# nextpyp/cet_pick

Hardware: AMD Instinct MI355X
Metric: subtomograms/sec (MoCo-3D train) + voxels/sec (heatmap+NMS) at 1/2/4/8 GPU (higher is better)
Workload: dtype f32; 1 GPU; moco_main.py moco3d_18: 3D encoder, synthetic 512x512x128 tomogram, 32^3 subtomo crops, batch 64 per GPU, r=1024, dim=128, m=0.999, T=0.1, SGD lr 1e-3; global_batch=64, parallelism=dp1, hipgraph=True

## Files before the change

cet_pick_amd/_lib.py:

```python
import ctypes
import os

import torch

_HERE = os.path.dirname(os.path.abspath(__file__))
LIB_PATH = os.environ.get("CETPICK_HIP_LIB") or os.path.join(_HERE, "libcetpick_hip.so")

_c = ctypes
_P, _I, _F, _Z, _D, _L = _c.c_void_p, _c.c_int, _c.c_float, _c.c_size_t, _c.c_double, _c.c_long


class ConvGeom(ctypes.Structure):
    _fields_ = [(f, _I) for f in "N Di Hi Wi Ci Co kd kh kw stride pd ph pw dd dh dw".split()]


_G = _c.POINTER(ConvGeom)


class Aug2d3dRanges(ctypes.Structure):
    _fields_ = [(f, _F) for f in "flip_p angle_lo angle_hi erase_p scale_lo scale_hi ratio_lo ratio_hi".split()]


_R = _c.POINTER(Aug2d3dRanges)

# ... 32 lines not shown
    "mi_nms3d": (_I, [_P, _P, _I, _I, _I, _I, _I, _S]),
    "mi_decode_workspace_bytes": (_Z, [_I, _I, _I, _I]),
    "mi_decode_workspace_init": (_I, [_P, _Z, _S]),
    "mi_sigmoid_nms_topk": (_I, [_P, _P, _I, _I, _I, _I, _I, _I, _I, _P, _P, _P, _Z, _S]),
    "mi_gauss3d_sep": (_I, [_P, _P, _P, _I, _I, _I, _F, _S]),
    "mi_dog_pick_workspace_bytes": (_Z, [_I, _I, _I, _I]),
    "mi_dog_pick": (_I, [_P, _I, _I, _I, _P, _I, _I, _I, _I, _P, _P, _P, _P, _I, _P, _P, _Z, _S]),
    "mi_greedy_nms3d_workspace_bytes": (_Z, [_I, _I, _I]),
    "mi_greedy_nms3d": (_I, [_P, _I, _I, _I, _F, _F, _F, _P, _P, _P, _I, _P, _Z, _S]),
    "mi_crop_normalize": (_I, [_P, _I, _I, _I, _P, _I, _I, _I, _I, _I, _I, _P, _S]),
    "mi_crop_normalize_table": (_I, [_P, _P, _P, _P, _P, _c.c_int64, _I, _I, _I, _I, _I, _I, _P, _S]),
    "mi_u8_roundtrip_normalize": (_I, [_P, _P, _Z, _F, _F, _S]),
    "mi_aug2d_params": (_I, [_P, _c.c_int64, _c.c_uint64, _I, _I, _I] + [_F] * 7 + [_P, _S]),
    "mi_aug2d_apply": (_I, [_P, _c.c_int64, _I, _P, _P, _c.c_int64, _I, _F, _F, _P, _S]),
    "mi_aug2d3d_params": (_I, [_P, _c.c_int64, _c.c_uint64, _I, _I, _R, _R, _P, _S]),
    "mi_aug2d3d_apply": (_I, [_P, _P, _c.c_int64, _I, _P, _P, _P, _P, _c.c_int64, _I, _F, _F, _F, _F, _P, _S]),
    "mi_aug3d_params": (_I, [_P, _c.c_int64, _c.c_uint64, _I, _I, _I, _I, _R3, _P, _S]),
    "mi_aug3d_workspace_bytes": (_Z, [_c.c_int64, _I, _I]),
    "mi_aug3d_apply": (_I, [_P, _P, _P, _c.c_int64, _P, _P, _c.c_int64, _I, _I, _P, _P, _Z, _S]),
    "mi_tilt_patches": (_I, [_P, _I, _P, _P, _c.c_int64, _I, _I, _D, _D, _P, _P, _S]),
    "mi_semi_labels": (_I, [_P, _I, _I, _I, _P, _c.c_int64, _P, _I, _I, _S]),
    "mi_semi_pairs": (_I, [_P, _P, _I, _P, _P, _c.c_int64, _I, _I, _P, _P, _P, _S]),
    "mi_gauss2d_slices": (_I, [_P, _P, _P, _I, _I, _I, _F, _S]),
    "mi_rec_reorder": (_I, [_P, _I, _I, _I, _I, _I, _I, _P, _S]),
    "mi_vol_stats_workspace_bytes": (_Z, [_L, _L]),
    "mi_vol_stats": (_I, [_P, _L, _L, _P, _P, _Z, _S]),
    "mi_zscore": (_I, [_P, _P, _L, _L, _P, _S]),
    "mi_zscore_quantize_minmax": (_I, [_P, _P, _L, _L, _P, _D, _D, _I, _S]),
    "mi_conv_workspace_bytes": (_Z, [_G]),
    "mi_conv_fwd_f32": (_I, [_P, _P, _P, _P, _I, _I, _G, _P, _Z, _S]),
    "mi_conv_dgrad_f32": (_I, [_P, _P, _P, _P, _P, _G, _P, _Z, _S]),
    "mi_conv_wgrad_f32": (_I, [_P, _P, _P, _G, _P, _Z, _P, _S]),
    "mi_conv_wgrad_batch_f32": (_I, [_P, _P, _P, _P, _I, _G, _Z, _P, _S]),
    "mi_stem2d_fwd_bias_f32": (_I, [_P, _P, _P, _P, _I, _I, _I, _I, _S]),
    "mi_upconv_tail_fwd": (_I, [_P, _P, _P, _P, _P] + [_I] * 7 + [_S]),
    "mi_smallk_image_bytes": (_Z, [_I, _I]),
    "mi_smallk_prep": (_I, [_P, _P, _I, _I, _S]),
    "mi_smallk_fwd_f32": (_I, [_P, _P, _P, _P, _I, _L, _I, _I, _I, _L, _I, _S]),
    "mi_smallk_heads_fwd_f32": (_I, [_P, _P, _P, _P, _P, _I, _L, _I, _L, _I, _S]),
    "mi_splitk_reduce_batch": (_I, [_P, _P, _P, _P, _I, _S]),
    "mi_linear_fwd_f32": (_I, [_P, _P, _P, _P, _I, _I, _I, _P, _Z, _S]),
    "mi_conv3d_direct_wimg_bytes": (_Z, [_I]),
    "mi_conv3d_direct_workspace_bytes": (_Z, [_I, _I]),
    "mi_conv3d_direct_usable": (_I, [_I] * 9),
    "mi_conv3d_direct_prep": (_I, [_P, _P, _P, _P, _I, _S]),
    "mi_conv3d_direct_f32": (_I, [_P, _P, _P, _P, _P, _I, _I, _I, _I, _I, _I, _P, _Z, _S]),
    "mi_conv2d_p2d_usable": (_I, [_I] * 4),
    "mi_conv2d_p2d_wimg_bytes": (_Z, [_I]),
    "mi_conv2d_p2d_prep": (_I, [_P, _P, _P, _P, _I, _S]),
    "mi_conv2d_p2d_f32": (_I, [_P, _P, _P, _P, _P, _I, _I, _I, _I, _I, _S]),
    "mi_conv2d_p2d_wgrad_workspace_bytes": (_Z, [_I] * 4),
    "mi_conv2d_p2d_wgrad_f32": (_I, [_P, _P, _P, _I, _I, _I, _I, _P, _Z, _S]),
    "mi_conv2d_stem3_workspace_bytes": (_Z, [_I]),
    "mi_conv2d_stem3_fwd_f32": (_I, [_P, _P, _P, _I, _I, _I, _I, _S]),
    "mi_conv2d_stem3_wgrad_f32": (_I, [_P, _P, _P, _I, _I, _I, _I, _P, _Z, _S]),
    "mi_conv3d_cube2_workspace_bytes": (_Z, [_I, _I]),
    "mi_conv3d_cube2_usable": (_I, [_I] * 9),
    "mi_conv3d_cube2_f32": (_I, [_P, _P, _P, _P, _P, _I, _I, _I, _I, _P, _Z, _S]),
    "mi_conv_d32_kind": (_I, [_I] * 12),
    "mi_conv_d32_image_bytes": (_Z, [_I, _I]),
    "mi_conv_d64_image_bytes": (_Z, [_I, _I]),
    "mi_conv_d32_prep": (_I, [_P, _P, _I, _I, _S]),
    "mi_conv_d64_prep_co": (_I, [_P, _P, _I, _I, _I, _S]),
    "mi_conv_d32_1x1_fwd_f32": (_I, [_P, _P, _P, _P, _I, _I, _I, _I, _I, _I, _I, _S]),
    "mi_conv_d32_fwd_pool_f32": (_I, [_P, _P, _P, _P, _P] + [_I] * 7 + [_S]),
    "mi_conv_d32_fwd_pool_strided_f32": (_I, [_P, _P, _P, _P, _I, _P] + [_I] * 7 + [_S]),
# ... 245 lines not shown
```

cet_pick_amd/csrc/conv_direct3.hip:

```cpp
#include "common.h"
#include "bf16x3.h"
#include <type_traits>
#include <algorithm>

namespace {

using namespace bf3;

constexpr int C = 64;
constexpr int PLANE = 64;
constexpr int TZ = 2;
constexpr int PZ = TZ + 2;
constexpr int NV = PZ * PLANE;
constexpr int LEAD = 16;
constexpr int ZREC = 34;
constexpr int NREC = LEAD + NV + ZREC;
constexpr int ARR = NREC * 16;
constexpr int KS = C / 16;
constexpr int PL_BYTES = 2 * ARR;
constexpr int KS_BYTES = 3 * PL_BYTES;
constexpr int LDS_BYTES = KS * KS_BYTES;
constexpr int ZBASE = (LEAD + NV) * 16;
constexpr int WBLK = 1024;
constexpr int WSTEP = 2 * 3 * WBLK;
// ... 440 lines not shown
    u32x4 o[3];
    cut8(v, o);
    unsigned char* dst = img + (long)(((cb * KSn + ks) * NTAP + tap) * 2 + cw) * (3 * WBLK) + lane * 16;
    store_planes(dst, WBLK, o);
}
__global__ __launch_bounds__(256) void direct3_prep_kernel(PrepBatch b) {
    const int fmt = b.wide[blockIdx.y], idx = blockIdx.x * 256 + threadIdx.x;
    if (fmt == 1) { if (blockIdx.x < PREP_BLOCKS_WIDE) direct3s_prep_body(b.w[blockIdx.y], b.img[blockIdx.y], b.dgrad[blockIdx.y], idx); }
    else if (fmt == 2) { if (blockIdx.x < PREP_BLOCKS_WIDE) direct3_prep_body<128>(b.w[blockIdx.y], b.img[blockIdx.y], b.dgrad[blockIdx.y], idx); }
    else if (fmt == 3) direct3s256_prep_body(b.w[blockIdx.y], b.img[blockIdx.y], b.dgrad[blockIdx.y], idx);
    else if (blockIdx.x < PREP_BLOCKS) direct3_prep_body<C>(b.w[blockIdx.y], b.img[blockIdx.y], b.dgrad[blockIdx.y], idx);
}

constexpr int WG_SPLITS = 28;
constexpr int WROW = 64;
constexpr int WHALF = (PLANE + 1) * WROW;
constexpr int WPL = 2 * WHALF;
constexpr int WOP = 3 * WPL;
constexpr int WBUF = 2 * WOP;
constexpr int WZERO = PLANE * WROW;

constexpr int WG_MAXPROB = 4;
struct Direct3WgradParams {
    const float* x[WG_MAXPROB];
    const float* dy[WG_MAXPROB];
    float* slabs[WG_MAXPROB];
    int N, D;
    unsigned bytes;
    int nprob, splits;
    int H, W;
};

constexpr int W_HB = 3 * 2 * 8 * 128;
template <bool V4, int CT, bool TILED = false>
__global__ __launch_bounds__(512, 2) void direct3_wgrad_kernel(Direct3WgradParams p) {
    __shared__ __attribute__((aligned(16))) unsigned char lds[2 * WBUF + (TILED ? 2 * W_HB : 16)];
    unsigned char* const halo = lds + 2 * WBUF;
    static_assert(!TILED || (!V4 && CT == 64), "tiled planes: the 64-channel geometry");
    constexpr int NBLK = CT / 64;
    const int tid = threadIdx.x, lane = tid & 63;
    const int wave = __builtin_amdgcn_readfirstlane(tid >> 6);
    const int h = lane >> 5, l32 = lane & 31, i16 = lane & 15, g16 = (lane >> 4) & 1;
    const int kh = wave >> 2, wm = (wave >> 1) & 1, wn = wave & 1;
    const int per_grp = p.nprob * p.splits;
    const int grp = blockIdx.x / per_grp, rem = blockIdx.x % per_grp;
    const int pb = rem / p.splits, split = rem % p.splits, stride = p.splits;
    const int pair = grp % 9, chb = grp / 9;
    const int ci0 = (chb / NBLK) * 64, co0 = (chb % NBLK) * 64;
    const int dz = pair / 3, dy = pair % 3;
    const int tiles_x = TILED ? p.W >> 3 : 1, tiles = TILED ? (p.H >> 3) * tiles_x : 1;
    const int n_planes = p.N * p.D * tiles;

    const __amdgpu_buffer_rsrc_t xrs = rsrc(p.x[pb], p.bytes), yrs = rsrc(p.dy[pb], p.bytes);
    const int st_vox = tid >> 3, st_cg = tid & 7;
    const unsigned st_src = TILED ? 4u * (unsigned)(((st_vox >> 3) * p.W + (st_vox & 7)) * C + st_cg * 8)
                                  : 4u * (unsigned)(st_vox * CT + st_cg * 8);
    const int h_side = tid >> 8, h_row = (tid >> 5) & 7, h_c2 = tid & 31;
    const unsigned x_ch = 4u * (unsigned)ci0, y_ch = 4u * (unsigned)co0;
    const int zsh = V4 ? 0 : dz - 1;
    const int st_lds = (st_cg >> 2) * WHALF + st_vox * WROW + (st_cg & 3) * 16;
    auto next_plane = [&](int from) {
        if (V4) return from < n_planes ? from : -1;
        for (int pi = from; pi < n_planes; pi += stride) {
            const int zi = (pi / tiles) % p.D + dz - 1;
            if ((unsigned)zi < (unsigned)p.D) return pi;
        }
        return -1;
    };
    u32x4 ldx[2], ldy[2];
    u32x2 ldh = {0u, 0u};
    unsigned u_y, u_x, u_h;
    auto unit_offsets = [&](int pi) {
        if (pi < 0) { u_y = u_x = u_h = 0x80000000u; return; }
        if (!TILED) {
            u_y = 4u * (unsigned)((long)pi * PLANE * CT) + y_ch + st_src;
            u_x = 4u * (unsigned)((long)(pi + zsh) * PLANE * CT) + x_ch + st_src;
            u_h = 0x80000000u;
            return;
        }
        const int pl = pi / tiles, t = pi % tiles, y0 = (t / tiles_x) * 8, x0 = (t % tiles_x) * 8;
        u_y = 4u * (unsigned)((((long)pl * p.H + y0) * p.W + x0) * C) + st_src;
        const int xr = y0 + (st_vox >> 3) + dy - 1;
        u_x = (unsigned)xr < (unsigned)p.H
                  ? 4u * (unsigned)((((long)(pl + dz - 1) * p.H + xr) * p.W + x0 + (st_vox & 7)) * C + st_cg * 8) : 0x80000000u;
        const int hr = y0 + h_row + dy - 1, hc = h_side ? x0 + 8 : x0 - 1;
        u_h = ((unsigned)hr < (unsigned)p.H && (unsigned)hc < (unsigned)p.W)
                  ? 4u * (unsigned)((((long)(pl + dz - 1) * p.H + hr) * p.W + hc) * C + 2 * h_c2) : 0x80000000u;
    };
    auto stage_load = [&](int pi) {
        unit_offsets(pi);
        ldx[0] = __builtin_amdgcn_raw_buffer_load_b128(xrs, (int)u_x, 0, 0);
        ldx[1] = __builtin_amdgcn_raw_buffer_load_b128(xrs, (int)(u_x + 16u), 0, 0);
        ldy[0] = __builtin_amdgcn_raw_buffer_load_b128(yrs, (int)u_y, 0, 0);
        ldy[1] = __builtin_amdgcn_raw_buffer_load_b128(yrs, (int)(u_y + 16u), 0, 0);
        if (TILED) ldh = __builtin_amdgcn_raw_buffer_load_b64(xrs, (int)u_h, 0, 0);
    };
    unsigned hcu[3];
    auto halo_cut = [&]() {
        const unsigned a1 = rest(ldh[0]), b1 = rest(ldh[1]), a2 = rest(a1), b2 = rest(b1);
        hcu[0] = pack2(ldh[1], ldh[0]);
        hcu[1] = pack2(b1, a1);
        hcu[2] = pack2(b2, a2);
    };
    auto halo_store = [&](int buf) {
#pragma unroll
        for (int pl = 0; pl < 3; ++pl)
            *reinterpret_cast<unsigned*>(halo + buf * W_HB + ((pl * 2 + h_side) * 8 + h_row) * 128 + h_c2 * 4) = hcu[pl];
    };
    auto stage_store_unit = [&](int buf, int op) {
        float v[8];
#pragma unroll
        for (int e = 0; e < 4; ++e) {
// ... 1 lines not shown
            v[4 + e] = __uint_as_float(op ? ldy[1][e] : ldx[1][e]);
        }
        u32x4 o[3];
        cut8(v, o);
        unsigned char* dst = lds + buf * WBUF + op * WOP + st_lds;
#pragma unroll
        for (int pl = 0; pl < 3; ++pl) *reinterpret_cast<u32x4*>(dst + pl * WPL) = o[pl];
        if (TILED && op == 0) { halo_cut(); halo_store(buf); }
    };

    const int q4 = i16 >> 2;
    const int coloff = (16 * g16 + 4 * (i16 & 3)) * 2;
    const int b_base = wn * WHALF + (2 * kh * 16 + 8 * h + q4) * WROW + coloff;
    int a_sel[2][2];
#pragma unroll
    for (int lk = 0; lk < 2; ++lk)
#pragma unroll
        for (int hi = 0; hi < 2; ++hi) {
            const int v = 16 * (2 * kh + lk) + 8 * h + 4 * hi + q4;
            if (V4) {
                const int zi = (v >> 4) + dz - 1, yi = ((v >> 2) & 3) + dy - 1;
                a_sel[lk][hi] = wm * WHALF + (((unsigned)zi < 4u && (unsigned)yi < 4u) ? ((zi * 4 + yi) * 4 + (v & 3)) * WROW : WZERO) + coloff;
            } else if (TILED) {
                a_sel[lk][hi] = wm * WHALF + v * WROW + coloff;
            } else {
                const int yi = (v >> 3) + dy - 1;
                a_sel[lk][hi] = wm * WHALF + ((unsigned)yi < 8u ? (yi * 8 + (v & 7)) * WROW : WZERO) + coloff;
            }
        }
    int h_off[2];
#pragma unroll
    for (int lk = 0; lk < 2; ++lk) h_off[lk] = (2 * (2 * kh + lk) + h) * 128 + (32 * wm + l32) * 2;
    unsigned hl[2][2][3];

    f32x16 acc[3];
#pragma unroll
    for (int t = 0; t < 3; ++t)
#pragma unroll
        for (int r = 0; r < 16; ++r) acc[t][r] = 0.f;

    for (int i = tid; i < 2 * 2 * 3 * 2 * (WROW / 16); i += 512) {
        const int img = i / (WROW / 16), c16 = i % (WROW / 16);
        *reinterpret_cast<u32x4*>(lds + img * WHALF + WZERO + c16 * 16) = u32x4{0u, 0u, 0u, 0u};
    }

    int cur = next_plane(split);
    int nxt = cur >= 0 ? next_plane(cur + stride) : -1;
    stage_load(cur);
    if (cur >= 0) { stage_store_unit(0, 0); stage_store_unit(0, 1); }
    stage_load(nxt);
    __syncthreads();

    bf16x8 af[2][3][3], bfg[2][3];
    auto read_piece = [&](int buf, int lk, int j, auto SETc) {
        constexpr int SET = decltype(SETc)::value;
        const unsigned char* xb = lds + buf * WBUF;
        if (j < 3) {
            const unsigned char* yb = xb + WOP + b_base + lk * 16 * WROW + j * WPL;
            const bf16x4 lo = __builtin_amdgcn_ds_read_tr16_b64_v4bf16((lds_bf16x4*)(yb));
            const bf16x4 hi = __builtin_amdgcn_ds_read_tr16_b64_v4bf16((lds_bf16x4*)(yb + 4 * WROW));
            bfg[SET][j] = __builtin_shufflevector(lo, hi, 0, 1, 2, 3, 4, 5, 6, 7);
        } else {
            const int pl = j - 3;
            const bf16x4 lo = __builtin_amdgcn_ds_read_tr16_b64_v4bf16((lds_bf16x4*)(xb + pl * WPL + a_sel[lk][0]));
            const bf16x4 hi = __builtin_amdgcn_ds_read_tr16_b64_v4bf16((lds_bf16x4*)(xb + pl * WPL + a_sel[lk][1]));
            af[SET][1][pl] = __builtin_shufflevector(lo, hi, 0, 1, 2, 3, 4, 5, 6, 7);
            if (TILED) {
#pragma unroll
                for (int sd = 0; sd < 2; ++sd)
                    hl[SET][sd][pl] = *reinterpret_cast<const unsigned short*>(halo + buf * W_HB + ((pl * 2 + sd) * 8) * 128 + h_off[lk]);
// ... 11 lines not shown
    };
    auto derive = [&](int set, int dxv, int pl) {
        const u32x4 c = __builtin_bit_cast(u32x4, af[set][1][pl]);
        u32x4 o;
        if (dxv == 0) {
            o[0] = c[0] << 16;
#pragma unroll
            for (int j = 1; j < 4; ++j) o[j] = __builtin_amdgcn_alignbit(c[j], c[j - 1], 16);
            if (V4) o[2] &= HI16;
            if (TILED) o[0] |= hl[set][0][pl];
        } else {
#pragma unroll
            for (int j = 0; j < 3; ++j) o[j] = __builtin_amdgcn_alignbit(c[j + 1], c[j], 16);
            o[3] = c[3] >> 16;
            if (V4) o[1] &= 0x0000ffffu;
            if (TILED) o[3] |= hl[set][1][pl] << 16;
        }
        af[set][dxv][pl] = __builtin_bit_cast(bf16x8, o);
    };
    unsigned cu[3][8];
    auto cut_a = [&](int op, int e) {
        cu[0][e] = op ? ldy[e >> 2][e & 3] : ldx[e >> 2][e & 3];
        cu[1][e] = rest(cu[0][e]);
    };
    auto cut_b = [&](int e) { cu[2][e] = rest(cu[1][e]); };
    auto store_piece = [&](int buf, int op, int pl) {
        u32x4 o;
#pragma unroll
        for (int d = 0; d < 4; ++d) o[d] = pack2(cu[pl][2 * d + 1], cu[pl][2 * d]);
        *reinterpret_cast<u32x4*>(lds + buf * WBUF + op * WOP + st_lds + pl * WPL) = o;
    };

    int buf = 0;
    if (cur >= 0) {
#pragma unroll
        for (int i = 0; i < 3; ++i) read_pair(0, 0, i);
    }
    constexpr int DXO[3] = {1, 0, 2};
    while (cur >= 0) {
        const int nn = nxt >= 0 ? next_plane(nxt + stride) : -1;
        unit_offsets(nn);
        __builtin_amdgcn_sched_barrier(0);
#pragma unroll
        for (int lk = 0; lk < 2; ++lk) {
            const int op = lk;
#pragma unroll
            for (int m = 0; m < 18; ++m) {
                const int dxm = DXO[m / 6];
                acc[dxm] = __builtin_amdgcn_mfma_f32_32x32x16_bf16(af[lk][dxm][PA[m % 6]], bfg[lk][PB[m % 6]], acc[dxm], 0, 0, 0);
                if (m < 3) derive(lk, 0, m);
                if (m >= 6 && m < 9) derive(lk, 2, m - 6);
                if (m >= 2 && m < 10) cut_a(op, m - 2);
                if (m >= 3 && m < 11) cut_b(m - 3);
                if (m >= 11 && m < 14) store_piece(buf ^ 1, op, m - 11);
                if (lk == 1 && m >= 14) {
                    const int i = m - 14, hf = i & 1;
                    if (i < 2) ldx[hf] = __builtin_amdgcn_raw_buffer_load_b128(xrs, (int)(u_x + 16u * hf), 0, 0);
                    else ldy[hf] = __builtin_amdgcn_raw_buffer_load_b128(yrs, (int)(u_y + 16u * hf), 0, 0);
                    if (TILED && i == 3) ldh = __builtin_amdgcn_raw_buffer_load_b64(xrs, (int)u_h, 0, 0);
                }
                if (TILED && lk == 0 && m == 14) halo_cut();
                if (TILED && lk == 0 && m == 15) halo_store(buf ^ 1);
                if (lk == 0) {
                    if (m < 3) read_pair(buf, 1, m);
                } else {
                    if (m == 13) __syncthreads();
// ... 307 lines not shown
    MI_RETURN_IF_LAUNCH_FAILED();
    return MI_OK;
}
int mi_direct3h_launch(const float* a, const void* wimg, float* out, const float* res, const float* mask, int relu, int N,
                       int D, int H, int W, hipStream_t s) {
    Direct3hParams p = {a, (const unsigned char*)wimg, out, res, mask, relu, N, D, H, W, (unsigned)(4l * N * D * H * W * C)};
    hipLaunchKernelGGL(direct3h_kernel, dim3((unsigned)((long)N * (D / TZ) * ((H + 7) / 8) * ((W + 7) / 8))), dim3(256), 0, s, p);
    MI_RETURN_IF_LAUNCH_FAILED();
    return MI_OK;
}
int mi_direct3_launch128(const float* a, const void* wimg, float* out, const float* res, const float* mask, int relu, int N,
                         int D, hipStream_t s) {
    Direct3Params p = {a, (const unsigned char*)wimg, out, res, mask, relu, N, D, (unsigned)(4l * N * D * PLANE * 128)};
    hipLaunchKernelGGL((direct3_kernel<true, 128>), dim3((unsigned)(N * (D / TZ)), 2), dim3(256), 0, s, p);
    MI_RETURN_IF_LAUNCH_FAILED();
    return MI_OK;
}

int mi_direct3s_launch(const float* a, const void* wimg, float* out, const float* res, const float* mask, int relu, int N,
                       hipStream_t s) {
    Direct3sParams p = {a, (const unsigned char*)wimg, out, res, mask, relu, N, (unsigned)(4l * N * VS * CS)};
    hipLaunchKernelGGL(direct3s_kernel<CS>, dim3((unsigned)(4 * N)), dim3(256), 0, s, p);
    MI_RETURN_IF_LAUNCH_FAILED();
    return MI_OK;
}
int mi_direct3s_launch256(const float* a, const void* wimg, float* out, const float* res, const float* mask, int relu, int N,
                          hipStream_t s) {
    Direct3sParams p = {a, (const unsigned char*)wimg, out, res, mask, relu, N, (unsigned)(4l * N * VS * 256)};
    hipLaunchKernelGGL(direct3s_kernel<256>, dim3((unsigned)(8 * N)), dim3(256), 0, s, p);
    MI_RETURN_IF_LAUNCH_FAILED();
    return MI_OK;
}

size_t mi_direct3_wgrad_slab_bytes() { return sizeof(float) * (size_t)WG_SPLITS * NTAP * C * C; }
int mi_direct3_wgrad_splits() { return WG_SPLITS; }

int mi_direct3_wgrad_launch(const float* x, const float* dy, float* slabs, int N, int D, hipStream_t s) {
    Direct3WgradParams p = {};
    p.x[0] = x; p.dy[0] = dy; p.slabs[0] = slabs; p.N = N; p.D = D; p.bytes = (unsigned)(4l * N * D * PLANE * C);
    p.nprob = 1; p.splits = WG_SPLITS;
    hipLaunchKernelGGL((direct3_wgrad_kernel<false, 64>), dim3(9 * WG_SPLITS), dim3(512), 0, s, p);
    MI_RETURN_IF_LAUNCH_FAILED();
    return MI_OK;
}
int mi_direct3_wgrad_batch_max() { return WG_MAXPROB; }
constexpr int WG_BATCH_SPLITS = 7;
int mi_direct3_wgrad_batch_splits(int nb) {
    if (nb < 1 || nb > WG_MAXPROB) return 0;
    if (const char* v = getenv("MI_D3W_BATCH_SPLITS")) { const int sv = atoi(v); if (sv >= 1 && sv <= WG_SPLITS) return sv; }
    return WG_BATCH_SPLITS;
}
int mi_direct3_wgrad_launch_batch(const float* const* xs, const float* const* dys, float* const* slabs, int nb, int N, int D,
                                  hipStream_t s) {
    if (nb < 1 || nb > WG_MAXPROB) return MI_E_ARG;
    Direct3WgradParams p = {};
    for (int i = 0; i < nb; ++i) { p.x[i] = xs[i]; p.dy[i] = dys[i]; p.slabs[i] = slabs[i]; }
    p.N = N; p.D = D; p.bytes = (unsigned)(4l * N * D * PLANE * C);
    p.nprob = nb; p.splits = mi_direct3_wgrad_batch_splits(nb);
    hipLaunchKernelGGL((direct3_wgrad_kernel<false, 64>), dim3(9 * nb * p.splits), dim3(512), 0, s, p);
    MI_RETURN_IF_LAUNCH_FAILED();
    return MI_OK;
}

constexpr int WS_SPLITS = 7, WS_BATCH_SPLITS = 2;
size_t mi_direct3s_wgrad_slab_bytes() { return sizeof(float) * (size_t)WS_SPLITS * NTAP * CS * CS; }
int mi_direct3s_wgrad_splits(int nb) {
    if (nb < 1 || nb > WG_MAXPROB) return 0;
    if (nb == 1) return WS_SPLITS;
    if (const char* v = getenv("MI_D3SW_BATCH_SPLITS")) { const int sv = atoi(v); if (sv >= 1 && sv <= WS_SPLITS) return sv; }
    return WS_BATCH_SPLITS;
}
int mi_direct3s_wgrad_launch_batch(const float* const* xs, const float* const* dys, float* const* slabs, int nb, int N, hipStream_t s) {
    if (nb < 1 || nb > WG_MAXPROB || N < 1) return MI_E_ARG;
    Direct3WgradParams p = {};
    for (int i = 0; i < nb; ++i) { p.x[i] = xs[i]; p.dy[i] = dys[i]; p.slabs[i] = slabs[i]; }
    p.N = N; p.D = 1; p.bytes = (unsigned)(4l * N * PLANE * CS);
    p.nprob = nb; p.splits = mi_direct3s_wgrad_splits(nb);
    hipLaunchKernelGGL((direct3_wgrad_kernel<true, 128>), dim3(36 * nb * p.splits), dim3(512), 0, s, p);
    MI_RETURN_IF_LAUNCH_FAILED();
    return MI_OK;
}

int mi_direct3t_wgrad_launch(const float* x, const float* dy, float* slabs, int N, int D, int H, int W, hipStream_t s) {
    if (H % 8 || W % 8 || H < 8 || W < 8) return MI_E_UNSUPPORTED;
    Direct3WgradParams p = {};
    p.x[0] = x; p.dy[0] = dy; p.slabs[0] = slabs; p.N = N; p.D = D; p.H = H; p.W = W;
    p.bytes = (unsigned)(4l * N * D * H * W * C);
    p.nprob = 1; p.splits = WG_SPLITS;
    hipLaunchKernelGGL((direct3_wgrad_kernel<false, 64, true>), dim3(9 * WG_SPLITS), dim3(512), 0, s, p);
    MI_RETURN_IF_LAUNCH_FAILED();
    return MI_OK;
}
// ... 45 lines not shown
```

cet_pick_amd/csrc/conv_igemm.hip:

```cpp
#include "common.h"
#include "bf16x3.h"
#include <algorithm>
#include <cstdlib>
#include <type_traits>

int mi_stem7_fwd(const float* x, const float* w, float* y, const float* res, int relu, int N, int D, int H, int W,
                 int Co, int bf16x3, void* ws, size_t ws_bytes, hipStream_t s, double* sums = nullptr);
size_t mi_stem7_fwd_workspace_bytes();
size_t mi_stem7_fwd_stats_workspace_bytes(int N, int D, int H, int W);
size_t mi_stem7_wgrad_workspace_bytes(int N, int D, int H, int W, int Co);
int mi_stem7_wgrad(const float* x, const float* dy, float* dw, int N, int D, int H, int W, int Co, int bf16x3, void* ws,
                   size_t ws_bytes, hipStream_t s);

int mi_direct3_kind(int N, int Di, int Hi, int Wi, int Ci, int Co, int kd, int kh, int kw, int stride, int pd, int ph,
                    int pw, int dd, int dh, int dw);
size_t mi_direct3_wimg_bytes(int channels);
size_t mi_direct3_slab_bytes(int N, int channels);
int mi_direct3_prep(const float* const* w, void* const* img, const int* dgrad, const int* channels, int n, hipStream_t s);
int mi_direct3_launch(const float* a, const void* wimg, float* out, const float* res, const float* mask, int relu, int N,
                      int D, hipStream_t s);
size_t mi_direct3_wimg_bytes_kind(int kind);
int mi_direct3_prep_kind(const float* const* w, void* const* img, const int* dgrad, const int* kinds, int n, hipStream_t s);
int mi_direct3s_launch256(const float* a, const void* wimg, float* out, const float* res, const float* mask, int relu, int N,
                          hipStream_t s);
int mi_direct3h_launch(const float* a, const void* wimg, float* out, const float* res, const float* mask, int relu, int N,
                       int D, int H, int W, hipStream_t s);
int mi_direct3_launch128(const float* a, const void* wimg, float* out, const float* res, const float* mask, int relu, int N,
                         int D, hipStream_t s);
int mi_direct3s_launch(const float* a, const void* wimg, float* out, const float* res, const float* mask, int relu, int N,
                       hipStream_t s);
int mi_direct3_finish_slabs(const float* slabs, int n_slabs, long out_elems, float* out, const float* res, const float* mask,
                            int relu, hipStream_t s);
size_t mi_direct3_wgrad_slab_bytes();
int mi_direct3_wgrad_splits();
int mi_direct3_wgrad_launch(const float* x, const float* dy, float* slabs, int N, int D, hipStream_t s);
int mi_direct3_wgrad_batch_max();
int mi_direct3_wgrad_batch_splits(int nb);
int mi_direct3_wgrad_launch_batch(const float* const* xs, const float* const* dys, float* const* slabs, int nb, int N, int D, hipStream_t s);
size_t mi_direct3s_wgrad_slab_bytes();
int mi_direct3s_wgrad_splits(int nb);
int mi_direct3s_wgrad_launch_batch(const float* const* xs, const float* const* dys, float* const* slabs, int nb, int N, hipStream_t s);
int mi_direct3t_wgrad_launch(const float* x, const float* dy, float* slabs, int N, int D, int H, int W, hipStream_t s);
int mi_direct3x_wgrad_splits(int kind);
size_t mi_direct3x_wgrad_slab_bytes(int kind);
int mi_direct3x_wgrad_launch(int kind, const float* x, const float* dy, float* slabs, int N, int D, hipStream_t s);
int mi_pair_wgrad_batch_max();
int mi_pair_wgrad_launch_batch(const float* const* xs, const float* const* dys, float* const* dws, float* const* slabs, int nb, int N, int Di,
                               int Ci, int Co, int k, int stride, hipStream_t s);
bool mi_cube2_usable(int N, int Di, int Hi, int Wi, int Ci, int Co, int kd, int kh, int kw, int stride, int pd, int ph, int pw,
                     int dd, int dh, int dw);
size_t mi_cube2_slab_bytes(int N, int C);
int mi_cube2_splits();
int mi_cube2_launch(int dgrad, const float* a, const float* w, float* slabs, int N, int C, hipStream_t s, const Cube2Final* fin = nullptr);
bool mi_pair_wgrad_usable(int N, int Di, int Hi, int Wi, int Ci, int Co, int kd, int kh, int kw, int stride, int pd, int ph, int pw,
                          int dd, int dh, int dw);
int mi_pair_wgrad_splits(int N, int Di, int Ci, int Co, int k, int stride);
size_t mi_pair_wgrad_slab_bytes(int N, int Di, int Ci, int Co, int k, int stride);
int mi_pair_wgrad_launch(const float* x, const float* dy, float* dwt, float* slabs, int N, int Di, int Ci, int Co, int k, int stride,
                         hipStream_t s);
bool mi_small_gemm_usable(long M, long N, long K);
int mi_small_gemm_launch(const float* a, long lda_m, long lda_k, long a_elems, const float* b, long ldb_k, long ldb_n,
                         long b_elems, const float* bias, float* c, int M, int N, int K, hipStream_t s,
                         const MiSmallGemmBN* bn = nullptr);

namespace {

using namespace bf3;

enum { MODE_FWD = 0, MODE_DGRAD = 1, MODE_WGRAD = 2 };
constexpr int NTHREADS = 256;
constexpr int MAX_CLASSES = 27;
// ... 1030 lines not shown
            if (rc || splits == 1) return rc;
            if (defer_splits) { *defer_splits = splits; return MI_OK; }
            return mi_direct3_finish_slabs((const float*)ws, splits, (long)g.kd * g.kh * g.kw * g.Ci * g.Co, out, nullptr, nullptr, 0, s);
        }
    }
    if (mode == MODE_WGRAD && dkind == 1 && ws && ws_bytes >= mi_direct3_wgrad_slab_bytes()) {
        g_last_conv_kernel = "direct3_wgrad + reduce";
        int rc = mi_direct3_wgrad_launch(a_src, b_src, (float*)ws, g.N, g.Di, s);
        if (rc) return rc;
        const int splits = mi_direct3_wgrad_splits();
        if (defer_splits) { *defer_splits = splits; return MI_OK; }
        const long out_elems = 27l * g.Ci * g.Co, n4 = out_elems / 4;
        hipLaunchKernelGGL(splitk_reduce_kernel, dim3((unsigned)std::min<long>((n4 + 255) / 256, 2048)), dim3(256), 0, s,
                           (const float*)ws, splits, out_elems, out, (const float*)nullptr, (const float*)nullptr, 0, n4);
        MI_RETURN_IF_LAUNCH_FAILED();
        return MI_OK;
    }
    if (mode == MODE_WGRAD && dkind == 2 && ws && ws_bytes >= mi_direct3s_wgrad_slab_bytes() && env_int("MI_D3S_WGRAD")) {
        g_last_conv_kernel = "direct3s_wgrad + reduce";
        const float* xs[1] = {a_src};
        const float* dys[1] = {b_src};
        float* sl[1] = {(float*)ws};
        int rc = mi_direct3s_wgrad_launch_batch(xs, dys, sl, 1, g.N, s);
        if (rc) return rc;
        const int splits = mi_direct3s_wgrad_splits(1);
        if (defer_splits) { *defer_splits = splits; return MI_OK; }
        return mi_direct3_finish_slabs((const float*)ws, splits, 27l * g.Ci * g.Co, out, nullptr, nullptr, 0, s);
    }
    if (mode == MODE_WGRAD && dkind == 5 && g.Hi % 8 == 0 && g.Wi % 8 == 0 && ws && ws_bytes >= mi_direct3_wgrad_slab_bytes() &&
        !env_int("MI_NO_D3T_WGRAD")) {
        g_last_conv_kernel = "direct3_wgrad (8 x 8 tiles) + reduce";
        int rc = mi_direct3t_wgrad_launch(a_src, b_src, (float*)ws, g.N, g.Di, g.Hi, g.Wi, s);
        if (rc) return rc;
        const int splits = mi_direct3_wgrad_splits();
        if (defer_splits) { *defer_splits = splits; return MI_OK; }
        return mi_direct3_finish_slabs((const float*)ws, splits, 27l * g.Ci * g.Co, out, nullptr, nullptr, 0, s);
    }
    if (mode == MODE_WGRAD && dkind == 3 && !env_int("MI_NO_D3X_WGRAD") && ws &&
        ws_bytes >= mi_direct3x_wgrad_slab_bytes(dkind)) {
        g_last_conv_kernel = "direct3_wgrad (128 channels) + reduce";
        int rc = mi_direct3x_wgrad_launch(dkind, a_src, b_src, (float*)ws, g.N, g.Di, s);
        if (rc) return rc;
        const int splits = mi_direct3x_wgrad_splits(dkind);
        if (defer_splits) { *defer_splits = splits; return MI_OK; }
        return mi_direct3_finish_slabs((const float*)ws, splits, 27l * g.Ci * g.Co, out, nullptr, nullptr, 0, s);
    }
    Setup st;
    int rc = setup_conv(mode, g, &st);
    if (rc) return rc;
    g_last_conv_kernel = st.pl.splits > 1 ? "implicit GEMM + reduce" : "implicit GEMM";
    ConvParams& p = st.p;
    Plan& pl = st.pl;
    p.a_src = a_src; p.b_src = b_src; p.res = res; p.mask = mask; p.relu = relu;
    p.res_bcast = res_bcast;
    const bool stem = (g.Ci == 1);
    const long out_elems = p.M * p.Ncols;
    if (pl.splits > 1) {
        size_t need = sizeof(float) * (size_t)out_elems * pl.splits;
        if (!ws || ws_bytes < need) pl.splits = 1;
    }
    p.splits = pl.splits;
    if (pl.splits > 1) { p.out = (float*)ws; p.slab_stride = out_elems; }
    else { p.out = out; p.slab_stride = 0; }
    {
        const int plan[PLAN_FIELDS] = {pl.bm, pl.bn, pl.bk, pl.splits, p.n_classes, p.border, p.fold,
                                       (p.wbox && g.Ci % pl.bm == 0) ? 1 : 0, (int)(pl.tiles_x * p.ny_tiles * pl.splits),
                                       plan_bf16x3(mode, stem, pl) ? 1 : 0, stem ? 1 : 0};
// ... 195 lines not shown
```

include/cetpick_hip.h:

```cpp
#ifndef CETPICK_HIP_H
#define CETPICK_HIP_H

#include <stddef.h>
#include <stdint.h>

#ifdef __cplusplus
extern "C" {
#endif

typedef void* mi_stream_t;

#define MI_OK 0
#define MI_E_ARG (-1)
#define MI_E_WORKSPACE (-2)
#define MI_E_UNSUPPORTED (-3)

int mi_abi_version(void);
int mi_graph_node_counts(void* graph, int* counts);
int mi_debug_stamp(void* slot, mi_stream_t stream);
const char* mi_debug_last_conv_kernel(void);
int mi_debug_last_conv_plan(int* out, int n);
const char* mi_build_arch(void);


// ... 77 lines not shown
                   const int64_t* sample_ids, const int32_t* table, int64_t n, int n_views, int crop, float* out,
                   void* workspace, size_t workspace_bytes, mi_stream_t stream);

typedef struct mi_tilt_desc {
    const float* tilts;
    const double* cos_sin;
    int32_t T, H, W, Zfull;
} mi_tilt_desc;
int mi_tilt_patches(const mi_tilt_desc* stacks, int n_stacks, const int32_t* owner, const int32_t* centres_xyz, int64_t n,
                    int cy, int cx, double bx, double by, float* out, uint8_t* valid, mi_stream_t stream);

int mi_semi_labels(float* hm, int D, int H, int W, const int32_t* centres_xyz, int64_t n, const float* stencil, int r,
                   int fill_unlabeled, mi_stream_t stream);
int mi_semi_pairs(const mi_vol_desc* tomos, const mi_vol_desc* labels, int n_tomos, const int32_t* owner,
                  const int32_t* centres_xyz, int64_t first, int n, int flip_y, float* input, float* input_aug, float* hm,
                  mi_stream_t stream);


typedef struct mi_conv_geom {
    int N, Di, Hi, Wi, Ci, Co, kd, kh, kw, stride, pd, ph, pw, dd, dh, dw;
} mi_conv_geom;

size_t mi_conv_workspace_bytes(const mi_conv_geom* g);
int mi_conv_fwd_f32(const float* x, const float* w, float* y, const float* res, int res_is_bias, int relu,
                    const mi_conv_geom* g, void* ws, size_t ws_bytes, mi_stream_t stream);
int mi_conv_dgrad_f32(const float* dy, const float* w, float* dx, const float* res, const float* mask,
                      const mi_conv_geom* g, void* ws, size_t ws_bytes, mi_stream_t stream);
int mi_conv_wgrad_f32(const float* x, const float* dy, float* dw, const mi_conv_geom* g, void* ws, size_t ws_bytes,
                      int* splits_out, mi_stream_t stream);
int mi_splitk_reduce_batch(const void* const* slabs, void* const* outs, const int* n_slabs, const long* out_elems, int n,
                           mi_stream_t stream);
int mi_conv_wgrad_batch_f32(const float* const* xs, const float* const* dys, float* const* dws, void* const* wss, int nb,
                            const mi_conv_geom* g, size_t ws_bytes, int* splits_out, mi_stream_t stream);

int mi_linear_bn_fwd_f32(const float* x, const float* w, const float* bias, float* xlin, float* y, int M, int Ci, int Co,
                         const float* gamma, const float* beta, float eps, float momentum, float* running_mean,
                         float* running_var, long long* num_batches_tracked, float* save_mean_invstd, int relu,
                         mi_stream_t stream);

int mi_linear_stats_fwd_f32(const float* x, const float* w, const float* bias, float* xlin, double* sums, int M, int Ci, int Co,
                            mi_stream_t stream);

size_t mi_conv3d_stem_stats_workspace_bytes(int N, int Di, int Hi, int Wi, int Co);
int mi_conv3d_stem_stats_f32(const float* x, const float* w, float* y, int N, int Di, int Hi, int Wi, int Co,
                             double* sums, void* ws, size_t ws_bytes, mi_stream_t stream);

int mi_linear_fwd_f32(const float* x, const float* w, const float* bias, float* y, int M, int Ci, int Co, void* ws,
                      size_t ws_bytes, mi_stream_t stream);

int mi_stem2d_fwd_bias_f32(const float* x, const float* w, const float* bias, float* y, int relu, int N, int H, int W,
                           mi_stream_t stream);
size_t mi_smallk_image_bytes(int K, int Co);
int mi_smallk_prep(const float* w, void* img, int K, int Co, mi_stream_t stream);
int mi_smallk_fwd_f32(const float* x, const void* img, const float* bias, float* y, int relu, long M, int Ci, int Co,
                      int ntaps, long plane, int D, mi_stream_t stream);
int mi_smallk_heads_fwd_f32(const float* x, const void* img, float* y_proj, const float* w_hm, float* y_hm, int k_hm, long M, int Ci,
                            long plane, int D, mi_stream_t stream);
size_t mi_conv3d_direct_wimg_bytes(int channels);
size_t mi_conv3d_direct_workspace_bytes(int N, int channels);
int mi_conv3d_direct_usable(int N, int Di, int Hi, int Wi, int Ci, int Co, int k, int stride, int pad);
int mi_conv3d_direct_prep(const void* const* w, void* const* img, const int* dgrad, const int* channels, int n,
                          mi_stream_t stream);
int mi_conv3d_direct_f32(const float* a, const void* wimg, float* out, const float* res, const float* mask, int relu,
                         int N, int Di, int Hi, int Wi, int channels, void* ws, size_t ws_bytes, mi_stream_t stream);

int mi_conv2d_p2d_usable(int N, int H, int W, int C);
// ... 293 lines not shown
```

Measured before the change: 41570 subtomograms/sec.

## Compute all dy taps per workgroup in direct3 wgrad to reuse staged planes

Adds a DZ variant of the 64-channel direct3 weight-gradient kernel where each workgroup owns one dz and accumulates all nine (dy,dx) taps, instead of one (dz,dy) pair per workgroup. Each staged x/dy plane is then reused across three dy offsets, which cuts global loads and LDS staging per MFMA. The cost is nine accumulator tiles, so occupancy drops to one workgroup per SIMD via launch bounds. Split counts are raised to keep the grid filled. The entry points are also exported as C API and the tiled path gets its own splits getter.

```diff
diff --git a/cet_pick_amd/_lib.py b/cet_pick_amd/_lib.py
--- a/cet_pick_amd/_lib.py
+++ b/cet_pick_amd/_lib.py
@@ -88,6 +88,11 @@
     "mi_conv_dgrad_f32": (_I, [_P, _P, _P, _P, _P, _G, _P, _Z, _S]),
     "mi_conv_wgrad_f32": (_I, [_P, _P, _P, _G, _P, _Z, _P, _S]),
     "mi_conv_wgrad_batch_f32": (_I, [_P, _P, _P, _P, _I, _G, _Z, _P, _S]),
+    "mi_direct3_wgrad_slab_bytes": (_Z, []),
+    "mi_direct3_wgrad_splits": (_I, []),
+    "mi_direct3_wgrad_batch_splits": (_I, [_I]),
+    "mi_direct3_wgrad_launch": (_I, [_P, _P, _P, _I, _I, _S]),
+    "mi_direct3_wgrad_launch_batch": (_I, [_P, _P, _P, _I, _I, _I, _S]),
     "mi_stem2d_fwd_bias_f32": (_I, [_P, _P, _P, _P, _I, _I, _I, _I, _S]),
     "mi_upconv_tail_fwd": (_I, [_P, _P, _P, _P, _P] + [_I] * 7 + [_S]),
     "mi_smallk_image_bytes": (_Z, [_I, _I]),
diff --git a/cet_pick_amd/csrc/conv_direct3.hip b/cet_pick_amd/csrc/conv_direct3.hip
--- a/cet_pick_amd/csrc/conv_direct3.hip
+++ b/cet_pick_amd/csrc/conv_direct3.hip
@@ -496,11 +496,12 @@
 };
 
 constexpr int W_HB = 3 * 2 * 8 * 128;
-template <bool V4, int CT, bool TILED = false>
-__global__ __launch_bounds__(512, 2) void direct3_wgrad_kernel(Direct3WgradParams p) {
+template <bool V4, int CT, bool TILED = false, bool DZ = false>
+__global__ __launch_bounds__(512, DZ ? 1 : 2) void direct3_wgrad_kernel(Direct3WgradParams p) {
     __shared__ __attribute__((aligned(16))) unsigned char lds[2 * WBUF + (TILED ? 2 * W_HB : 16)];
     unsigned char* const halo = lds + 2 * WBUF;
     static_assert(!TILED || (!V4 && CT == 64), "tiled planes: the 64-channel geometry");
+    static_assert(!DZ || (!V4 && CT == 64 && !TILED), "one workgroup per dz: 64 channels on 8 x 8 planes");
     constexpr int NBLK = CT / 64;
     const int tid = threadIdx.x, lane = tid & 63;
     const int wave = __builtin_amdgcn_readfirstlane(tid >> 6);
@@ -509,7 +510,7 @@
     const int per_grp = p.nprob * p.splits;
     const int grp = blockIdx.x / per_grp, rem = blockIdx.x % per_grp;
     const int pb = rem / p.splits, split = rem % p.splits, stride = p.splits;
-    const int pair = grp % 9, chb = grp / 9;
+    const int pair = DZ ? 3 * grp + 1 : grp % 9, chb = DZ ? 0 : grp / 9;
     const int ci0 = (chb / NBLK) * 64, co0 = (chb % NBLK) * 64;
     const int dz = pair / 3, dy = pair % 3;
     const int tiles_x = TILED ? p.W >> 3 : 1, tiles = TILED ? (p.H >> 3) * tiles_x : 1;
@@ -535,13 +536,13 @@
     u32x2 ldh = {0u, 0u};
     unsigned u_y, u_x, u_h;
     auto unit_offsets = [&](int pi) {
-        if (pi < 0) { u_y = u_x = u_h = 0x80000000u; return; }
         if (!TILED) {
-            u_y = 4u * (unsigned)((long)pi * PLANE * CT) + y_ch + st_src;
-            u_x = 4u * (unsigned)((long)(pi + zsh) * PLANE * CT) + x_ch + st_src;
+            u_y = pi < 0 ? 0x80000000u : 4u * (unsigned)((long)pi * PLANE * CT) + y_ch + st_src;
+            u_x = pi < 0 ? 0x80000000u : 4u * (unsigned)((long)(pi + zsh) * PLANE * CT) + x_ch + st_src;
             u_h = 0x80000000u;
             return;
         }
+        if (pi < 0) { u_y = u_x = u_h = 0x80000000u; return; }
         const int pl = pi / tiles, t = pi % tiles, y0 = (t / tiles_x) * 8, x0 = (t % tiles_x) * 8;
         u_y = 4u * (unsigned)((((long)pl * p.H + y0) * p.W + x0) * C) + st_src;
         const int xr = y0 + (st_vox >> 3) + dy - 1;
@@ -609,10 +610,17 @@
 #pragma unroll
     for (int lk = 0; lk < 2; ++lk) h_off[lk] = (2 * (2 * kh + lk) + h) * 128 + (32 * wm + l32) * 2;
     unsigned hl[2][2][3];
-
-    f32x16 acc[3];
-#pragma unroll
-    for (int t = 0; t < 3; ++t)
+    int a_top[2], a_bot[2];
+#pragma unroll
+    for (int hi = 0; hi < 2; ++hi) {
+        a_top[hi] = (kh == 0 && h == 0) ? wm * WHALF + WZERO + coloff : a_sel[0][hi] - 8 * WROW;
+        a_bot[hi] = (kh == 1 && h == 1) ? wm * WHALF + WZERO + coloff : a_sel[1][hi] + 8 * WROW;
+    }
+
+    constexpr int NACC = DZ ? 9 : 3;
+    f32x16 acc[NACC];
+#pragma unroll
+    for (int t = 0; t < NACC; ++t)
 #pragma unroll
         for (int r = 0; r < 16; ++r) acc[t][r] = 0.f;
 
@@ -690,6 +698,98 @@
     };
 
     int buf = 0;
+    (void)a_top; (void)a_bot;
+    if constexpr (DZ) {
+        auto read_a = [&](int b, auto STEPc, int pl) {
+            constexpr int step = decltype(STEPc)::value, lk = step / 3, dyv = step % 3, SET = step & 1;
+            const unsigned char* xb = lds + b * WBUF + pl * WPL;
+            const int o0 = (dyv == 0 && lk == 0) ? a_top[0] : (dyv == 2 && lk == 1) ? a_bot[0] : a_sel[lk][0] + (dyv - 1) * 8 * WROW;
+            const int o1 = (dyv == 0 && lk == 0) ? a_top[1] : (dyv == 2 && lk == 1) ? a_bot[1] : a_sel[lk][1] + (dyv - 1) * 8 * WROW;
+            const bf16x4 lo = __builtin_amdgcn_ds_read_tr16_b64_v4bf16((lds_bf16x4*)(xb + o0));
+            const bf16x4 hi = __builtin_amdgcn_ds_read_tr16_b64_v4bf16((lds_bf16x4*)(xb + o1));
+            af[SET][1][pl] = __builtin_shufflevector(lo, hi, 0, 1, 2, 3, 4, 5, 6, 7);
+        };
+        auto step_body = [&](auto STEPc) {
+            constexpr int step = decltype(STEPc)::value, lk = step / 3, dyv = step % 3, set = step & 1;
+            constexpr int DXO[3] = {1, 0, 2}, BP[3] = {0, 2, 1}, AP[3] = {2, 0, 1};
+#pragma unroll
+            for (int m = 0; m < 18; ++m) {
+                const int dxm = DXO[m / 6];
+                acc[dyv * 3 + dxm] = __builtin_amdgcn_mfma_f32_32x32x16_bf16(af[set][dxm][PA[m % 6]], bfg[lk][PB[m % 6]], acc[dyv * 3 + dxm], 0, 0, 0);
+                if (m < 3) derive(set, 0, m);
+                if (m >= 6 && m < 9) derive(set, 2, m - 6);
+                if (step < 2) {
+                    if (m >= 2 && m < 10) cut_a(step, m - 2);
+                    if (m >= 3 && m < 11) cut_b(m - 3);
+                    if (m >= 11 && m < 14) store_piece(buf ^ 1, step, m - 11);
+                }
+                if (step == 3 && m >= 14) {
+                    const int i = m - 14, hf = i & 1;
+                    if (i < 2) ldx[hf] = __builtin_amdgcn_raw_buffer_load_b128(xrs, (int)(u_x + 16u * hf), 0, 0);
+                    else ldy[hf] = __builtin_amdgcn_raw_buffer_load_b128(yrs, (int)(u_y + 16u * hf), 0, 0);
+                }
+                if (step == 2 && m >= 3 && m < 6) read_piece(buf, 1, BP[m - 3], std::integral_constant<int, 1>{});
+                if (step < 5) {
+                    if (m >= 10 && m < 13) read_a(buf, std::integral_constant<int, (step + 1) % 6>{}, AP[m - 10]);
+                } else {
+                    if (m == 9) __syncthreads();
+                    if (m >= 10 && m < 13 && nxt >= 0) {
+                        read_piece(buf ^ 1, 0, BP[m - 10], std::integral_constant<int, 0>{});
+                        read_a(buf ^ 1, std::integral_constant<int, 0>{}, AP[m - 10]);
+                    }
+                }
+                __builtin_amdgcn_sched_barrier(0);
+            }
+        };
+        if (cur >= 0) {
+            constexpr int BP[3] = {0, 2, 1}, AP[3] = {2, 0, 1};
+#pragma unroll
+            for (int i = 0; i < 3; ++i) {
+                read_piece(0, 0, BP[i], std::integral_constant<int, 0>{});
+                read_a(0, std::integral_constant<int, 0>{}, AP[i]);
+            }
+        }
+        while (cur >= 0) {
+            const int nn = nxt >= 0 ? next_plane(nxt + stride) : -1;
+            unit_offsets(nn);
+            __builtin_amdgcn_sched_barrier(0);
+            step_body(std::integral_constant<int, 0>{});
+            step_body(std::integral_constant<int, 1>{});
+            step_body(std::integral_constant<int, 2>{});
+            step_body(std::integral_constant<int, 3>{});
+            step_body(std::integral_constant<int, 4>{});
+            step_body(std::integral_constant<int, 5>{});
+            buf ^= 1;
+            cur = nxt;
+            nxt = nn;
+        }
+        __syncthreads();
+        float* red = reinterpret_cast<float*>(lds);
+        float* out = p.slabs[pb] + (long)split * (NTAP * CT * CT);
+#pragma unroll
+        for (int dyv = 0; dyv < 3; ++dyv) {
+            if (kh == 1) {
+#pragma unroll
+                for (int dx = 0; dx < 3; ++dx)
+#pragma unroll
+                    for (int r = 0; r < 16; ++r) red[(((wave & 3) * 3 + dx) * 16 + r) * 64 + lane] = acc[dyv * 3 + dx][r];
+            }
+            __syncthreads();
+            if (kh == 0) {
+#pragma unroll
+                for (int dx = 0; dx < 3; ++dx) {
+                    const int tap = (dz * 3 + dyv) * 3 + dx;
+#pragma unroll
+                    for (int r = 0; r < 16; ++r) {
+                        const int ci = 32 * wm + (r & 3) + 8 * (r >> 2) + 4 * h;
+                        out[((long)tap * CT + ci) * CT + 32 * wn + l32] = acc[dyv * 3 + dx][r] + red[((wave * 3 + dx) * 16 + r) * 64 + lane];
+                    }
+                }
+            }
+            if (dyv < 2) __syncthreads();
+        }
+        return;
+    }
     if (cur >= 0) {
 #pragma unroll
         for (int i = 0; i < 3; ++i) read_pair(0, 0, i);
@@ -1063,32 +1163,39 @@
     return MI_OK;
 }
 
-size_t mi_direct3_wgrad_slab_bytes() { return sizeof(float) * (size_t)WG_SPLITS * NTAP * C * C; }
-int mi_direct3_wgrad_splits() { return WG_SPLITS; }
-
-int mi_direct3_wgrad_launch(const float* x, const float* dy, float* slabs, int N, int D, hipStream_t s) {
+constexpr int WG_DZ_SPLITS = 84, WG_DZ_BATCH_SPLITS = 10;
+constexpr int WG_MAX_SPLITS = WG_DZ_SPLITS > WG_SPLITS ? WG_DZ_SPLITS : WG_SPLITS;
+extern "C" size_t mi_direct3_wgrad_slab_bytes() { return sizeof(float) * (size_t)WG_MAX_SPLITS * NTAP * C * C; }
+extern "C" int mi_direct3_wgrad_splits() { return WG_DZ_SPLITS; }
+int mi_direct3t_wgrad_splits() { return WG_SPLITS; }
+static bool d3w_extent_ok(int N, int D) { return N >= 1 && D >= 1 && 4l * N * D * PLANE * C < (1l << 31); }
+
+extern "C" int mi_direct3_wgrad_launch(const float* x, const float* dy, float* slabs, int N, int D, mi_stream_t stream) {
+    if (!x || !dy || !slabs) return MI_E_ARG;
+    if (!d3w_extent_ok(N, D)) return MI_E_UNSUPPORTED;
     Direct3WgradParams p = {};
     p.x[0] = x; p.dy[0] = dy; p.slabs[0] = slabs; p.N = N; p.D = D; p.bytes = (unsigned)(4l * N * D * PLANE * C);
-    p.nprob = 1; p.splits = WG_SPLITS;
-    hipLaunchKernelGGL((direct3_wgrad_kernel<false, 64>), dim3(9 * WG_SPLITS), dim3(512), 0, s, p);
+    p.nprob = 1; p.splits = WG_DZ_SPLITS;
+    hipLaunchKernelGGL((direct3_wgrad_kernel<false, 64, false, true>), dim3(3 * WG_DZ_SPLITS), dim3(512), 0, (hipStream_t)stream, p);
     MI_RETURN_IF_LAUNCH_FAILED();
     return MI_OK;
 }
 int mi_direct3_wgrad_batch_max() { return WG_MAXPROB; }
-constexpr int WG_BATCH_SPLITS = 7;
-int mi_direct3_wgrad_batch_splits(int nb) {
+extern "C" int mi_direct3_wgrad_batch_splits(int nb) {
     if (nb < 1 || nb > WG_MAXPROB) return 0;
-    if (const char* v = getenv("MI_D3W_BATCH_SPLITS")) { const int sv = atoi(v); if (sv >= 1 && sv <= WG_SPLITS) return sv; }
-    return WG_BATCH_SPLITS;
-}
-int mi_direct3_wgrad_launch_batch(const float* const* xs, const float* const* dys, float* const* slabs, int nb, int N, int D,
-                                  hipStream_t s) {
-    if (nb < 1 || nb > WG_MAXPROB) return MI_E_ARG;
+    if (const char* v = getenv("MI_D3W_BATCH_SPLITS")) { const int sv = atoi(v); if (sv >= 1 && sv <= WG_MAX_SPLITS) return sv; }
+    return WG_DZ_BATCH_SPLITS;
+}
+extern "C" int mi_direct3_wgrad_launch_batch(const float* const* xs, const float* const* dys, float* const* slabs, int nb, int N, int D,
+                                             mi_stream_t stream) {
+    if (!xs || !dys || !slabs || nb < 1 || nb > WG_MAXPROB) return MI_E_ARG;
+    for (int i = 0; i < nb; ++i) if (!xs[i] || !dys[i] || !slabs[i]) return MI_E_ARG;
+    if (!d3w_extent_ok(N, D)) return MI_E_UNSUPPORTED;
     Direct3WgradParams p = {};
     for (int i = 0; i < nb; ++i) { p.x[i] = xs[i]; p.dy[i] = dys[i]; p.slabs[i] = slabs[i]; }
     p.N = N; p.D = D; p.bytes = (unsigned)(4l * N * D * PLANE * C);
     p.nprob = nb; p.splits = mi_direct3_wgrad_batch_splits(nb);
-    hipLaunchKernelGGL((direct3_wgrad_kernel<false, 64>), dim3(9 * nb * p.splits), dim3(512), 0, s, p);
+    hipLaunchKernelGGL((direct3_wgrad_kernel<false, 64, false, true>), dim3(3 * nb * p.splits), dim3(512), 0, (hipStream_t)stream, p);
     MI_RETURN_IF_LAUNCH_FAILED();
     return MI_OK;
 }
diff --git a/cet_pick_amd/csrc/conv_igemm.hip b/cet_pick_amd/csrc/conv_igemm.hip
--- a/cet_pick_amd/csrc/conv_igemm.hip
+++ b/cet_pick_amd/csrc/conv_igemm.hip
@@ -31,12 +31,8 @@
                        hipStream_t s);
 int mi_direct3_finish_slabs(const float* slabs, int n_slabs, long out_elems, float* out, const float* res, const float* mask,
                             int relu, hipStream_t s);
-size_t mi_direct3_wgrad_slab_bytes();
-int mi_direct3_wgrad_splits();
-int mi_direct3_wgrad_launch(const float* x, const float* dy, float* slabs, int N, int D, hipStream_t s);
 int mi_direct3_wgrad_batch_max();
-int mi_direct3_wgrad_batch_splits(int nb);
-int mi_direct3_wgrad_launch_batch(const float* const* xs, const float* const* dys, float* const* slabs, int nb, int N, int D, hipStream_t s);
+int mi_direct3t_wgrad_splits();
 size_t mi_direct3s_wgrad_slab_bytes();
 int mi_direct3s_wgrad_splits(int nb);
 int mi_direct3s_wgrad_launch_batch(const float* const* xs, const float* const* dys, float* const* slabs, int nb, int N, hipStream_t s);
@@ -1133,7 +1129,7 @@
         g_last_conv_kernel = "direct3_wgrad (8 x 8 tiles) + reduce";
         int rc = mi_direct3t_wgrad_launch(a_src, b_src, (float*)ws, g.N, g.Di, g.Hi, g.Wi, s);
         if (rc) return rc;
-        const int splits = mi_direct3_wgrad_splits();
+        const int splits = mi_direct3t_wgrad_splits();
         if (defer_splits) { *defer_splits = splits; return MI_OK; }
         return mi_direct3_finish_slabs((const float*)ws, splits, 27l * g.Ci * g.Co, out, nullptr, nullptr, 0, s);
     }
diff --git a/include/cetpick_hip.h b/include/cetpick_hip.h
--- a/include/cetpick_hip.h
+++ b/include/cetpick_hip.h
@@ -133,6 +133,12 @@
                            mi_stream_t stream);
 int mi_conv_wgrad_batch_f32(const float* const* xs, const float* const* dys, float* const* dws, void* const* wss, int nb,
                             const mi_conv_geom* g, size_t ws_bytes, int* splits_out, mi_stream_t stream);
+size_t mi_direct3_wgrad_slab_bytes(void);
+int mi_direct3_wgrad_splits(void);
+int mi_direct3_wgrad_batch_splits(int nb);
+int mi_direct3_wgrad_launch(const float* x, const float* dy, float* slabs, int N, int D, mi_stream_t stream);
+int mi_direct3_wgrad_launch_batch(const float* const* xs, const float* const* dys, float* const* slabs, int nb, int N, int D,
+                                  mi_stream_t stream);
 
 int mi_linear_bn_fwd_f32(const float* x, const float* w, const float* bias, float* xlin, float* y, int M, int Ci, int Co,
                          const float* gamma, const float* beta, float eps, float momentum, float* running_mean,
```

Measured after the change: 41600 subtomograms/sec, median of 3. No clear change (+0.1%).
